# flxrcz/hommx

Measured on AMD Instinct MI355X. Metric: micro-cell solves/sec, higher is better.
Workload: dtype f64

## Files before the change

### hommx_amd/csrc/fused2d.hip

```cpp
#include <hip/hip_runtime.h>
#include <stdint.h>

#include <type_traits>

#include "kernels.h"
#include "sweep_acc.h"

#ifndef HOMMX_FUSED_WAVES_PER_SIMD
#define HOMMX_FUSED_WAVES_PER_SIMD 2
#endif

namespace hommx {

typedef double d4 __attribute__((ext_vector_type(4)));
typedef double d2 __attribute__((ext_vector_type(2)));

__device__ __forceinline__ double uniform_f64(double v) {
  return __hiloint2double(__builtin_amdgcn_readfirstlane(__double2hiint(v)),
                          __builtin_amdgcn_readfirstlane(__double2loint(v)));
}

struct CoefRow {
  double a0, a1;
  double a0m, a1m;
};

constexpr int MATP = 48;

template <int NB>
struct alignas(16) Lds {
  double mat[(NB + 1) * MATP];
  double ubuf[4 * NB];
  double tsc[16 * 17];
  double rrow[2][NB];
  double vrow[2][NB];
  double vnat[2][NB];
  double e0row[NB];
  double e1row[NB];
  double e0nat[NB];
  double e1nat[NB];
  double dgnat[NB];
  double cenat[NB + 2];
};
template <int NB>
struct alignas(16) LdsIso {
  static constexpr int PARK = NB == 32 ? 12 * 64 : 0;
  double ubuf[4 * NB];
  double tsc[16 * 17];
  double rrow[2][NB];
  double vrow[2][NB];
  double vnat[2][NB];
  double e0row[NB];
  double e0nat[NB];
  double dgnat[NB];
  double cenat[NB + 2];
  double park[PARK ? PARK : 1];
};

struct NoFact {};
template <int NB, bool FACT, bool ISO>
__global__ __launch_bounds__(64, (NB == 32 && ISO) ? 3 : HOMMX_FUSED_WAVES_PER_SIMD) void k_poisson2d_fused(
    const double* __restrict__ coef, const double* __restrict__ Mmat, double* __restrict__ out,
    int32_t* __restrict__ info, int n, long long ncells, const CoefSource src, std::conditional_t<FACT, double*, NoFact> fact
#ifdef HOMMX_FUSED_DEBUG
    , double* __restrict__ dbg
#endif
) {
  constexpr int NT = NB / 16, KK = NB / 4, CG = 64 / NB;
  constexpr int P = MATP;
  constexpr bool PARK = ISO && NB == 32;
  static_assert(!(FACT && ISO), "the factor record keeps the general path");
  __shared__ std::conditional_t<ISO, LdsIso<NB>, Lds<NB>> L;

  const long long cell = blockIdx.x;
  if (cell >= ncells) return;
  __builtin_assume(n >= 3);
  __builtin_assume(n <= NB);
  const int l = threadIdx.x;
  const int j = l & 15, k = l >> 4;
  const int c = l % NB, g = l / NB;
  const int lb = l - c;
  const int p0 = NB - n;
  const bool valid = c >= p0;
  const int cn = c - p0;
  const int cm = valid ? (c == p0 ? NB - 1 : c - 1) : c;
  const int cp = valid ? (c == NB - 1 ? p0 : c + 1) : c;
  const int prow = (c & 3) * KK + (c >> 2);

  const int ownB = (k + 1) * P + j;
  [[maybe_unused]] int leftB[NT];
#pragma unroll
  for (int tj = 0; tj < NT; ++tj) {
    const int col = 16 * tj + j;
    leftB[tj] = (k + 1) * P + (col == p0 ? NB - 1 : col - 1);
  }
#define OWN(ti, tj, r) (ownB + (16 * (ti) + 4 * (r)) * P + 16 * (tj))
#define LEFT(ti, tj, r) (leftB[tj] + (16 * (ti) + 4 * (r)) * P)
  [[maybe_unused]] unsigned matOff = 0;
  if constexpr (!ISO) matOff = accl::lds_offset(&L.mat[0]);
  [[maybe_unused]] const unsigned haloA = matOff + 8u * (unsigned)(p0 * P + j);

  const int mode = src.mode;
  const unsigned char* mask = static_cast<const unsigned char*>(src.table);
  const double* table = static_cast<const double*>(src.table);
  const double* cc = mode == COEF_STREAM ? coef + cell * (2ll * n * n) : coef + cell * 2;
  constexpr int NL = NB * NB / 64;
  double2 pv[NL];
  if (mode == COEF_STREAM) {
#pragma unroll
    for (int i = 0; i < NL; ++i) {
      const int el = 2 * l + 128 * i;
      pv[i] = el < 2 * n * n ? *reinterpret_cast<const double2*>(cc + el) : double2{0.0, 0.0};
    }
  }

  if constexpr (!ISO)
    for (int i = l; i < (NB + 1) * P; i += 64) L.mat[i] = 0.0;
  if (l == 0) L.cenat[0] = 0.0;

  double m00 = 1.0, m01 = 0.0, m10 = 0.0, m11 = 1.0;
  if (!ISO && Mmat) {
    const double* mp = Mmat + cell * 4;
    m00 = mp[0]; m01 = mp[1]; m10 = mp[2]; m11 = mp[3];
  }
  const double al = ISO ? 0.5 : uniform_f64(0.5 * (m00 * m00 + m10 * m10));
  const double be = ISO ? 0.5 : uniform_f64(0.5 * (m01 * m01 + m11 * m11));
  const double ga = ISO ? 0.0 : uniform_f64(0.5 * (m00 * m01 + m10 * m11));
  const double ab = ISO ? 1.0 : uniform_f64(al - 2.0 * ga + be);

  double ph0 = 0.0, ph1 = 0.0;
  if (mode != COEF_STREAM) {
    ph0 = cc[0];
    ph1 = cc[1];
  }
  const int nq = src.nq;
  auto sample = [&](long long el) {
    double acc = 0.0;
    for (int q = 0; q < nq; ++q)
      acc = add_rn(acc, mul_rn(src.weights[q], div_rn(1.0, add_rn(ph0, mul_rn(ph1, table[el * nq + q])))));
    return acc;
  };
  auto load_pair = [&](long long el, double& a0, double& a1) {
    if (mode == COEF_TWO_PHASE) {
      const uchar2 mk = *reinterpret_cast<const uchar2*>(mask + el);
      a0 = mk.x ? ph1 : ph0;
      a1 = mk.y ? ph1 : ph0;
    } else if (mode == COEF_AFFINE) {
      const double2 g2 = *reinterpret_cast<const double2*>(table + el);
      a0 = add_rn(ph0, mul_rn(ph1, g2.x));
      a1 = add_rn(ph0, mul_rn(ph1, g2.y));
    } else if (mode == COEF_RECIPROCAL) {
      a0 = sample(el);
      a1 = sample(el + 1);
    } else {
      const double2 v = *reinterpret_cast<const double2*>(cc + el);
      a0 = v.x; a1 = v.y;
    }
  };
  int esh;
  {
    int ef = 0;
    if (mode == COEF_STREAM) {
      int hm = 0;
#pragma unroll
      for (int i = 0; i < NL; ++i) hm = max(hm, max(__double2hiint(pv[i].x) & 0x7fffffff, __double2hiint(pv[i].y) & 0x7fffffff));
      ef = hm >> 20;
    } else {
      for (long long el = 2 * l; el < 2ll * n * n; el += 128) {
        double a0, a1;
        load_pair(el, a0, a1);
        const int f0 = (__double2hiint(a0) >> 20) & 0x7ff, f1 = (__double2hiint(a1) >> 20) & 0x7ff;
        ef = max(ef, max(f0, f1));
      }
    }
#pragma unroll
    for (int off = 32; off >= 1; off >>= 1) ef = max(ef, __shfl_xor(ef, off, 64));
    const int fm = (__double2hiint(6.0 * (al + be)) >> 20) & 0x7ff;
    const int sh = (ef == 0 || ef == 0x7ff ? 0 : ef - 1023) + (fm == 0 || fm == 0x7ff ? 0 : fm - 1023) + 2;
    esh = __builtin_amdgcn_readfirstlane(ef == 0 || ef == 0x7ff ? 0 : sh);
  }
  auto load_row = [&](int jc) {
    CoefRow r;
    r.a0 = 0.0; r.a1 = 0.0;
    if (valid) {
      load_pair(2 * (jc * n + cn), r.a0, r.a1);
      r.a0 = ldexp(r.a0, -esh);
      r.a1 = ldexp(r.a1, -esh);
    }
    r.a0m = __shfl(r.a0, lb + cm, 64);
    r.a1m = __shfl(r.a1, lb + cm, 64);
    return r;
  };
  auto st_diag = [&](const CoefRow& cur, const CoefRow& prev) {
    return valid ? cur.a0 * al + cur.a1 * be + cur.a0m * ab + prev.a0m * be + prev.a1m * al + prev.a1 * ab : 1.0;
  };
  auto st_E = [&](const CoefRow& cur, const CoefRow& prev) { return (cur.a0 + prev.a1) * (ga - al); };
  auto st_N = [&](const CoefRow& cur) { return (cur.a1 + cur.a0m) * (ga - be); };
  auto st_NE = [&](const CoefRow& cur) { return -ga * (cur.a0 + cur.a1); };
  auto st_p0 = [&](const CoefRow& cur, const CoefRow& prev) { return cur.a0 - cur.a0m - prev.a1m + prev.a1; };
  auto st_p1 = [&](const CoefRow& cur, const CoefRow& prev) { return cur.a1 + cur.a0m - prev.a0m - prev.a1; };

  [[maybe_unused]] auto band_write = [&](double dv, double ov, bool sym, bool clear) {
    if constexpr (!ISO) {
      if (g == 0) {
        const double d_ = clear ? 0.0 : dv, o_ = clear ? 0.0 : ov;
        L.mat[(c + 1) * P + c] = d_;
        if (valid) {
          L.mat[(cp + 1) * P + c] = o_;
          if (sym) L.mat[(c + 1) * P + cp] = o_;
        }
      }
    }
  };
  auto sub_band = [&](double (&x)[NT][NT][4], const double (&dgq)[NT], const double (&ceq)[NT], const double (&cemq)[NT]) {
#pragma unroll
    for (int t = 0; t < NT; ++t) {
      using namespace accl;
#define DIAG_LO(r) (OneLane<0, 4 * (r)>::lo | OneLane<1, 4 * (r) + 1>::lo | OneLane<2, 4 * (r) + 2>::lo | OneLane<3, 4 * (r) + 3>::lo)
#define DIAG_HI(r) (OneLane<0, 4 * (r)>::hi | OneLane<1, 4 * (r) + 1>::hi | OneLane<2, 4 * (r) + 2>::hi | OneLane<3, 4 * (r) + 3>::hi)
      masked_sub4<DIAG_LO(0), DIAG_HI(0), DIAG_LO(1), DIAG_HI(1), DIAG_LO(2), DIAG_HI(2), DIAG_LO(3), DIAG_HI(3)>(
          x[t][t][0], x[t][t][1], x[t][t][2], x[t][t][3], dgq[t]);
#define SUB_LO(r) (((r) ? OneLane<0, (4 * (r) - 1) & 15>::lo : 0u) | OneLane<1, 4 * (r)>::lo | OneLane<2, 4 * (r) + 1>::lo | OneLane<3, 4 * (r) + 2>::lo)
#define SUB_HI(r) (((r) ? OneLane<0, (4 * (r) - 1) & 15>::hi : 0u) | OneLane<1, 4 * (r)>::hi | OneLane<2, 4 * (r) + 1>::hi | OneLane<3, 4 * (r) + 2>::hi)
      masked_sub4<SUB_LO(0), SUB_HI(0), SUB_LO(1), SUB_HI(1), SUB_LO(2), SUB_HI(2), SUB_LO(3), SUB_HI(3)>(
          x[t][t][0], x[t][t][1], x[t][t][2], x[t][t][3], ceq[t]);
#define SUP_LO(r) (OneLane<0, 4 * (r) + 1>::lo | OneLane<1, 4 * (r) + 2>::lo | OneLane<2, 4 * (r) + 3>::lo | ((r) < 3 ? OneLane<3, (4 * (r) + 4) & 15>::lo : 0u))
#define SUP_HI(r) (OneLane<0, 4 * (r) + 1>::hi | OneLane<1, 4 * (r) + 2>::hi | OneLane<2, 4 * (r) + 3>::hi | ((r) < 3 ? OneLane<3, (4 * (r) + 4) & 15>::hi : 0u))
      masked_sub4<SUP_LO(0), SUP_HI(0), SUP_LO(1), SUP_HI(1), SUP_LO(2), SUP_HI(2), SUP_LO(3), SUP_HI(3)>(
          x[t][t][0], x[t][t][1], x[t][t][2], x[t][t][3], cemq[t]);
#undef DIAG_LO
#undef DIAG_HI
#undef SUB_LO
#undef SUB_HI
#undef SUP_LO
#undef SUP_HI
    }
    if (NT == 2) {
      using namespace accl;
      masked_sub<OneLane<0, 15>::lo, OneLane<0, 15>::hi>(x[NT - 1][0][0], ceq[0]);
      masked_sub<OneLane<3, 0>::lo, OneLane<3, 0>::hi>(x[0][NT - 1][3], cemq[NT - 1]);
    }
  };
  [[maybe_unused]] auto band_regs = [&](double (&x)[NT][NT][4], double dv, double ov) {
    double dq[NT], oq[NT], omq[NT];
#pragma unroll
    for (int tj = 0; tj < NT; ++tj) {
      const int col = 16 * tj + j;
      dq[tj] = __shfl(dv, col, 64);
      oq[tj] = __shfl(ov, col, 64);
      const double om = __shfl(ov, (col + 63) & 63, 64);
      omq[tj] = col == 0 ? 0.0 : om;
    }
#pragma unroll
    for (int ti = 0; ti < NT; ++ti)
#pragma unroll
      for (int tj = 0; tj < NT; ++tj)
#pragma unroll
        for (int r = 0; r < 4; ++r) x[ti][tj][r] = 0.0;
    sub_band(x, dq, oq, omq);
    const double cw = readlane_f64(ov, NB - 1);
#pragma unroll
    for (int tj = 0; tj < NT; ++tj) x[NT - 1][tj][3] = (k == 3 && 16 * tj + j == p0) ? x[NT - 1][tj][3] - cw : x[NT - 1][tj][3];
#pragma unroll
    for (int ti = 0; ti < NT; ++ti)
#pragma unroll
      for (int r = 0; r < 4; ++r) x[ti][NT - 1][r] = (j == 15 && 16 * ti + 4 * r + k == p0) ? x[ti][NT - 1][r] - cw : x[ti][NT - 1][r];
  };

  [[maybe_unused]] double* rec = nullptr;
  if constexpr (FACT) rec = fact + cell * fused_fact_doubles(n);
  [[maybe_unused]] double* srec = nullptr;
  if constexpr (FACT) srec = rec + fused_fact_header(NB);

  double wf[NT][KK];
  double a[NT][NT][4];
  d4 slr[NT][NT];
  double rr[2];
  double rlm;
  CoefRow cur;
  double asum;
  __syncthreads();
  {
    const CoefRow rowA = load_row(n - 2);
    const CoefRow rowB = load_row(n - 1);
    cur = load_row(0);
    asum = (rowB.a0 + rowB.a1) + (cur.a0 + cur.a1);
    if constexpr (FACT) {
      const double neB = st_NE(rowB);
      const double c1 = __shfl(neB, lb + cm, 64);
      if (g == 0) {
        rec[c] = st_N(rowB);
        rec[NB + c] = c1;
      }
      if (l < 4) rec[4 * NB + l] = l == 0 ? m00 : l == 1 ? m01 : l == 2 ? m10 : m11;
      if (l == 4) rec[4 * NB + 4] = (double)esh;
    }
    if constexpr (ISO) {
      band_regs(a, -st_diag(rowB, rowA), -st_E(rowB, rowA));
#pragma unroll
      for (int ti = 0; ti < NT; ++ti)
#pragma unroll
        for (int tj = 0; tj <= ti; ++tj)
#pragma unroll
          for (int r = 0; r < 4; ++r) slr[ti][tj][r] = a[ti][tj][r];
      if constexpr (PARK) {
#pragma unroll
        for (int ti = 0; ti < NT; ++ti)
#pragma unroll
          for (int tj = 0; tj <= ti; ++tj)
#pragma unroll
            for (int r = 0; r < 4; ++r) L.park[(4 * (ti * (ti + 1) / 2 + tj) + r) * 64 + l] = slr[ti][tj][r];
      }
      band_regs(a, st_diag(cur, rowB), st_E(cur, rowB));
      const double dv = st_N(rowB);
#pragma unroll
      for (int t = 0; t < NT; ++t) {
        using namespace accl;
#pragma unroll
        for (int kk = 0; kk < KK; ++kk) wf[t][kk] = 0.0;
        const double dq = __shfl(dv, 16 * t + j, 64);
        amov<DiagMask<0>::lo, DiagMask<0>::hi>(wf[t][4 * t], dq);
        amov<DiagMask<1>::lo, DiagMask<1>::hi>(wf[t][4 * t + 1], dq);
        amov<DiagMask<2>::lo, DiagMask<2>::hi>(wf[t][4 * t + 2], dq);
        amov<DiagMask<3>::lo, DiagMask<3>::hi>(wf[t][4 * t + 3], dq);
      }
    } else {
    {
      const double dv = st_diag(rowB, rowA), ov = st_E(rowB, rowA);
      band_write(dv, ov, true, false);
      __syncthreads();
#pragma unroll
      for (int ti = 0; ti < NT; ++ti)
#pragma unroll
        for (int tj = 0; tj <= ti; ++tj)
#pragma unroll
          for (int r = 0; r < 4; ++r) slr[ti][tj][r] = L.mat[OWN(ti, tj, r)];
      __syncthreads();
      band_write(dv, ov, true, true);
      __syncthreads();
    }
    {
      const double dv = st_N(rowB), ov = st_NE(rowB);
      band_write(dv, ov, false, false);
      __syncthreads();
#pragma unroll
      for (int t = 0; t < NT; ++t)
#pragma unroll
        for (int kk = 0; kk < KK; ++kk) wf[t][kk] = L.mat[OWN(kk >> 2, t, kk & 3)];
      __syncthreads();
      band_write(dv, ov, false, true);
      __syncthreads();
    }
    {
      const double dv = -st_diag(cur, rowB), ov = -st_E(cur, rowB);
      band_write(dv, ov, true, false);
      __syncthreads();
#pragma unroll
      for (int ti = 0; ti < NT; ++ti)
#pragma unroll
        for (int tj = 0; tj < NT; ++tj)
#pragma unroll
          for (int r = 0; r < 4; ++r) a[ti][tj][r] = L.mat[OWN(ti, tj, r)];
      __syncthreads();
      band_write(dv, ov, true, true);
      __syncthreads();
    }
    }
    rr[0] = st_p0(cur, rowB); rr[1] = st_p1(cur, rowB);
    rlm = (k >> 1) ? st_p1(rowB, rowA) : st_p0(rowB, rowA);
  }
  double ga_ = 0.0, gb_ = 0.0;
  int bad = 0, badstep = 0;
  [[maybe_unused]] double wselR[NT];
#pragma unroll
  for (int tj = 0; tj < NT; ++tj) wselR[tj] = (k == 3 && 16 * tj + j == p0) ? 1.0 : 0.0;
  [[maybe_unused]] const double wselC = (j == 15 && k == (p0 & 3)) ? 1.0 : 0.0;
  [[maybe_unused]] const int laneR = 48 + (p0 & 15), tileR = p0 >> 4, laneC = 16 * (p0 & 3) + 15;
  double indw[KK];
#pragma unroll
  for (int q = 0; q < KK; ++q) indw[q] = uniform_f64((q == (p0 >> 2)) ? 1.0 : 0.0);

  for (int jr = 0; jr <= n - 2; ++jr) {
    const bool lastStep = (jr == n - 2);
    CoefRow nxt = cur;
    if (!lastStep) {
      nxt = load_row(jr + 1);
      asum += nxt.a0 + nxt.a1;
    }
    const double e0c = st_N(cur);
    [[maybe_unused]] double neC = 0.0, e1c = 0.0;
    if constexpr (!ISO) {
      neC = st_NE(cur);
      e1c = __shfl(neC, lb + cm, 64);
    }
    if (lastStep) {
      if constexpr (ISO) {
#pragma unroll
        for (int t = 0; t < NT; ++t) {
          using namespace accl;
          const double me = -__shfl(e0c, 16 * t + j, 64);
          masked_sub4<DiagMask<0>::lo, DiagMask<0>::hi, DiagMask<1>::lo, DiagMask<1>::hi, DiagMask<2>::lo, DiagMask<2>::hi, DiagMask<3>::lo,
                      DiagMask<3>::hi>(wf[t][4 * t], wf[t][4 * t + 1], wf[t][4 * t + 2], wf[t][4 * t + 3], me);
        }
      } else {
        for (int i = l; i < (NB + 1) * P; i += 64) L.mat[i] = 0.0;
        __syncthreads();
        if (g == 0) {
          L.mat[(c + 1) * P + c] = e0c;
          if (valid) L.mat[(c + 1) * P + cp] = neC;
        }
        __syncthreads();
#pragma unroll
        for (int t = 0; t < NT; ++t)
#pragma unroll
          for (int kk = 0; kk < KK; ++kk) wf[t][kk] += L.mat[OWN(kk >> 2, t, kk & 3)];
        __syncthreads();
      }
    }
    [[maybe_unused]] double pn0 = 0.0, pn1 = 0.0;
    if constexpr (ISO) {
      pn0 = st_p0(nxt, cur);
      pn1 = st_p1(nxt, cur);
    }
    const double dgc = st_diag(nxt, cur), cec = st_E(nxt, cur);
    if (g == 0) {
      L.rrow[0][prow] = rr[0];
      L.rrow[1][prow] = rr[1];
      L.e0row[prow] = e0c;
      if constexpr (!ISO) L.e1row[prow] = e1c;
      L.e0nat[c] = e0c;
      if constexpr (!ISO) L.e1nat[c] = e1c;
      L.dgnat[c] = dgc;
      L.cenat[1 + c] = cec;
    }

    {
      int badj = 0;
#ifdef HOMMX_FUSED_SWEEP32
      accl::Sweep<NB>::run(a, L.ubuf, j, k, badj);
#else
      __builtin_amdgcn_s_setprio(1);
      if constexpr (NB == 32) accl::block_inverse32(a, L.ubuf, L.tsc, j, k, badj);
      else accl::Sweep<NB>::run(a, L.ubuf, j, k, badj);
      __builtin_amdgcn_s_setprio(0);
#endif
      if (badj && !bad) { bad = 1; badstep = jr + 1; }
    }
    if constexpr (FACT) {
#pragma unroll
      for (int ti = 0; ti < NT; ++ti)
#pragma unroll
        for (int tj = 0; tj < NT; ++tj)
#pragma unroll
          for (int r = 0; r < 4; ++r) srec[((ti * NT + tj) * 4 + r) * 64 + l] = a[ti][tj][r];
      if (g == 0) {
        srec[NB * NB + 2 * NB + c] = e0c;
        srec[NB * NB + 3 * NB + c] = e1c;
      }
    }
#ifdef HOMMX_FUSED_DEBUG
    if (dbg && cell == 0) {
      double* q = dbg + (size_t)jr * 4 * NB * NB;
#pragma unroll
      for (int ti = 0; ti < NT; ++ti)
#pragma unroll
        for (int tj = 0; tj < NT; ++tj)
#pragma unroll
          for (int r = 0; r < 4; ++r) q[(16 * ti + 4 * r + k) * NB + 16 * tj + j] = a[ti][tj][r];
#pragma unroll
      for (int t = 0; t < NT; ++t)
#pragma unroll
        for (int kk = 0; kk < KK; ++kk) q[NB * NB + (16 * t + j) * NB + 4 * kk + k] = wf[t][kk];
    }
#endif

    if constexpr (!ISO) if (!lastStep) {
#pragma unroll
      for (int ti = 0; ti < NT; ++ti)
#pragma unroll
        for (int tj = 0; tj < NT; ++tj)
#pragma unroll
          for (int r = 0; r < 4; ++r) L.mat[OWN(ti, tj, r)] = a[ti][tj][r];
#pragma unroll
      for (int tj = 0; tj < NT; ++tj)
        accl::masked_lds_store<accl::RowMask<3>::lo, accl::RowMask<3>::hi>(haloA + 128u * tj, a[NT - 1][tj][3]);
    }

    d4 vt[NT][NT];
#pragma unroll
    for (int x = 0; x < NT; ++x)
#pragma unroll
      for (int y = 0; y < NT; ++y) vt[x][y] = d4{0.0, 0.0, 0.0, 0.0};
#pragma unroll
    for (int kk = 0; kk < KK; ++kk)
#pragma unroll
      for (int x = 0; x < NT; ++x)
#pragma unroll
        for (int y = 0; y < NT; ++y)
          vt[x][y] = __builtin_amdgcn_mfma_f64_16x16x4f64(a[kk >> 2][x][kk & 3], wf[y][kk], vt[x][y], 0, 0, 0);

    if constexpr (PARK) {
#pragma unroll
      for (int x = 0; x < NT; ++x)
#pragma unroll
        for (int y = 0; y <= x; ++y) {
          double* pk = &L.park[4 * (x * (x + 1) / 2 + y) * 64 + l];
          d4 s;
#pragma unroll
          for (int r = 0; r < 4; ++r) s[r] = pk[64 * r];
#pragma unroll
          for (int kk = 0; kk < KK; ++kk) s = __builtin_amdgcn_mfma_f64_16x16x4f64(vt[kk >> 2][x][kk & 3], wf[y][kk], s, 0, 0, 0);
#pragma unroll
          for (int r = 0; r < 4; ++r) pk[64 * r] = s[r];
        }
    } else {
#pragma unroll
    for (int kk = 0; kk < KK; ++kk)
#pragma unroll
      for (int x = 0; x < NT; ++x)
#pragma unroll
        for (int y = 0; y <= x; ++y)
          slr[x][y] = __builtin_amdgcn_mfma_f64_16x16x4f64(vt[kk >> 2][x][kk & 3], wf[y][kk], slr[x][y], 0, 0, 0);
    }

    double z;
    {
      double part[2][NT];
#pragma unroll
      for (int m = 0; m < 2; ++m)
#pragma unroll
        for (int tj = 0; tj < NT; ++tj) part[m][tj] = 0.0;
#pragma unroll
      for (int m = 0; m < 2; ++m)
#pragma unroll
        for (int ti = 0; ti < NT; ++ti) {
          const d4 q = *reinterpret_cast<const d4*>(&L.rrow[m][k * KK + 4 * ti]);
#pragma unroll
          for (int r = 0; r < 4; ++r)
#pragma unroll
            for (int tj = 0; tj < NT; ++tj) part[m][tj] = fma(q[r], a[ti][tj][r], part[m][tj]);
        }
      if (NT == 2) {
        double s_[2];
#pragma unroll
        for (int m = 0; m < 2; ++m) {
          double x = part[m][0], y = part[m][NT - 1];
          swap16(x, y);
          s_[m] = x + y;
        }
        swap32(s_[0], s_[1]);
        z = s_[0] + s_[1];
      } else {
        double x = part[0][0], y = part[1][0];
        swap32(x, y);
        z = add_xor16(x + y);
      }
    }
    if constexpr (ISO) {
      ga_ = fma(z, L.rrow[0][prow], ga_);
      gb_ = fma(z, L.rrow[1][prow], gb_);
    } else {
      ga_ = fma(z, rr[0], ga_);
      gb_ = fma(z, rr[1], gb_);
    }
    L.vnat[k >> 1][c] = z;
    L.vrow[k >> 1][prow] = z;
    if constexpr (FACT) {
      if (NB == 32 || !(k & 1)) srec[NB * NB + (k >> 1) * NB + c] = z;
      srec += fused_fact_step(NB);
    }

    {
      double part[2][NT];
#pragma unroll
      for (int m = 0; m < 2; ++m) {
        double v[KK];
#pragma unroll
        for (int q4 = 0; q4 < KK; q4 += 4) {
          const d4 q = *reinterpret_cast<const d4*>(&L.vrow[m][k * KK + q4]);
          v[q4] = q[0]; v[q4 + 1] = q[1]; v[q4 + 2] = q[2]; v[q4 + 3] = q[3];
        }
#pragma unroll
        for (int t = 0; t < NT; ++t) {
          double acc = 0.0;
#pragma unroll
          for (int kk = 0; kk < KK; ++kk) acc = fma(v[kk], wf[t][kk], acc);
          part[m][t] = acc;
        }
      }
      double z6;
      if (NT == 2) {
        double s_[2];
#pragma unroll
        for (int m = 0; m < 2; ++m) {
          double x = part[m][0], y = part[m][NT - 1];
          swap16(x, y);
          s_[m] = x + y;
        }
        swap32(s_[0], s_[1]);
        z6 = s_[0] + s_[1];
      } else {
        double x = part[0][0], y = part[1][0];
        swap32(x, y);
        z6 = add_xor16(x + y);
      }
      rlm += z6;
    }

    if (!lastStep) {
      [[maybe_unused]] double e0r[KK];
      [[maybe_unused]] double e1r[KK];
#pragma unroll
      for (int q4 = 0; q4 < KK; q4 += 4) {
        if constexpr (!ISO) {
          const d4 x = *reinterpret_cast<const d4*>(&L.e0row[k * KK + q4]);
          const d4 y = *reinterpret_cast<const d4*>(&L.e1row[k * KK + q4]);
          e0r[q4] = x[0]; e0r[q4 + 1] = x[1]; e0r[q4 + 2] = x[2]; e0r[q4 + 3] = x[3];
          e1r[q4] = y[0]; e1r[q4 + 1] = y[1]; e1r[q4 + 2] = y[2]; e1r[q4 + 3] = y[3];
        }
      }
      {
        double e0q[NT], dgq[NT], ceq[NT], cemq[NT];
        [[maybe_unused]] double e1q[NT];
#pragma unroll
        for (int tj = 0; tj < NT; ++tj) {
          e0q[tj] = L.e0nat[16 * tj + j];
          if constexpr (!ISO) e1q[tj] = L.e1nat[16 * tj + j];
          dgq[tj] = L.dgnat[16 * tj + j];
          ceq[tj] = L.cenat[1 + 16 * tj + j];
          cemq[tj] = L.cenat[16 * tj + j];
        }
#pragma unroll
        for (int ti = 0; ti < NT; ++ti)
#pragma unroll
          for (int r = 0; r < 4; ++r)
#pragma unroll
            for (int tj = 0; tj < NT; ++tj) {
              if constexpr (ISO) {
                a[ti][tj][r] = -(L.e0row[k * KK + 4 * ti + r] * (e0q[tj] * a[ti][tj][r]));
              } else {
                const double nl = L.mat[LEFT(ti, tj, r)];
                const double nu = L.mat[OWN(ti, tj, r) - P];
                const double nul = L.mat[LEFT(ti, tj, r) - P];
                const double x = fma(e1q[tj], nl, e0q[tj] * a[ti][tj][r]);
                const double xu = fma(e1q[tj], nul, e0q[tj] * nu);
                a[ti][tj][r] = -fma(e0r[4 * ti + r], x, e1r[4 * ti + r] * xu);
              }
            }
        sub_band(a, dgq, ceq, cemq);
        {
          const double cw = readlane_f64(cec, NB - 1);
#pragma unroll
          for (int tj = 0; tj < NT; ++tj) {
            if constexpr (ISO) a[NT - 1][tj][3] = (l == laneR && tj == tileR) ? fma(-cw, 1.0, a[NT - 1][tj][3]) : fma(-cw, 0.0, a[NT - 1][tj][3]);
            else a[NT - 1][tj][3] = fma(-cw, wselR[tj], a[NT - 1][tj][3]);
          }
          double vcol;
          if constexpr (ISO) vcol = l == laneC ? -cw : -cw * 0.0;
          else vcol = -cw * wselC;
#pragma unroll
          for (int ti = 0; ti < NT; ++ti)
#pragma unroll
            for (int r = 0; r < 4; ++r) a[ti][NT - 1][r] = fma(vcol, indw[4 * ti + r], a[ti][NT - 1][r]);
        }
      }

      if constexpr (ISO) {
#pragma unroll
        for (int kk = 0; kk < KK; ++kk)
#pragma unroll
          for (int t = 0; t < NT; ++t) wf[t][kk] = L.e0row[k * KK + kk] * vt[kk >> 2][t][kk & 3];
      } else {
#pragma unroll
        for (int x = 0; x < NT; ++x)
#pragma unroll
          for (int y = 0; y < NT; ++y)
#pragma unroll
            for (int r = 0; r < 4; ++r) L.mat[OWN(x, y, r)] = vt[x][y][r];
#pragma unroll
        for (int y = 0; y < NT; ++y)
          accl::masked_lds_store<accl::RowMask<3>::lo, accl::RowMask<3>::hi>(haloA + 128u * y, vt[NT - 1][y][3]);
#pragma unroll
        for (int t = 0; t < NT; ++t)
#pragma unroll
          for (int kk = 0; kk < KK; ++kk) {
            const double up = L.mat[OWN(kk >> 2, t, kk & 3) - P];
            wf[t][kk] = fma(e1r[kk], up, e0r[kk] * vt[kk >> 2][t][kk & 3]);
          }
      }

      {
        const double v0 = L.vnat[0][c], v1 = L.vnat[1][c];
        if constexpr (ISO) {
          const double e0 = L.e0nat[c];
          rr[0] = fma(v0, e0, pn0);
          rr[1] = fma(v1, e0, pn1);
        } else {
          const double vm0 = L.vnat[0][cm], vm1 = L.vnat[1][cm];
          rr[0] = fma(vm0, e1c, fma(v0, e0c, st_p0(nxt, cur)));
          rr[1] = fma(vm1, e1c, fma(v1, e0c, st_p1(nxt, cur)));
        }
      }
      cur = nxt;
      __syncthreads();
    }
  }

  int lt = l, jt = j, kt = k, ct = c, prowt = prow;
  if constexpr (ISO) {
    lt = (int)__lane_id();
    asm volatile("" : "+v"(lt));
    jt = lt & 15;
    kt = lt >> 4;
    ct = lt % NB;
    prowt = (ct & 3) * KK + (ct >> 2);
  }
  {
  const int l = lt, j = jt, k = kt, c = ct, prow = prowt;
  [[maybe_unused]] auto bfly = [&](double v, int off) {
    const int ad = (l ^ off) << 2;
    return __hiloint2double(__builtin_amdgcn_ds_bpermute(ad, __double2hiint(v)), __builtin_amdgcn_ds_bpermute(ad, __double2loint(v)));
  };
  {
    if constexpr (PARK) {
#pragma unroll
      for (int ti = 0; ti < NT; ++ti)
#pragma unroll
        for (int tj = 0; tj <= ti; ++tj)
#pragma unroll
          for (int r = 0; r < 4; ++r) slr[ti][tj][r] = L.park[(4 * (ti * (ti + 1) / 2 + tj) + r) * 64 + l];
    }
    [[maybe_unused]] d4 sup = d4{0.0, 0.0, 0.0, 0.0};
    if (NT == 2) {
      if constexpr (ISO) {
        sup = accl::transpose_tile(slr[NT - 1][0], L.tsc, j, k);
      } else {
#pragma unroll
        for (int r = 0; r < 4; ++r) L.mat[OWN(1, 0, r)] = slr[NT - 1][0][r];
        __syncthreads();
      }
    }
#pragma unroll
    for (int ti = 0; ti < NT; ++ti)
#pragma unroll
      for (int tj = 0; tj < NT; ++tj)
#pragma unroll
        for (int r = 0; r < 4; ++r) {
          if (tj <= ti) a[ti][tj][r] = -slr[ti][tj][r];
          else if constexpr (ISO) a[ti][tj][r] = -sup[r];
          else a[ti][tj][r] = -L.mat[(16 + j + 1) * P + 4 * r + k];
        }
    {
      using namespace accl;
#pragma unroll
      for (int tj = 0; tj < NT; ++tj) amov<RowMask<3>::lo, RowMask<3>::hi>(a[NT - 1][tj][3], 0.0);
#pragma unroll
      for (int ti = 0; ti < NT; ++ti)
#pragma unroll
        for (int r = 0; r < 4; ++r) amov<ColMask<15>::lo, ColMask<15>::hi>(a[ti][NT - 1][r], 0.0);
      amov<OneLane<3, 15>::lo, OneLane<3, 15>::hi>(a[NT - 1][NT - 1][3], -1.0);
    }
    if (c == NB - 1) rlm = 0.0;
    __syncthreads();
    L.rrow[k >> 1][prow] = rlm;
    L.vnat[k >> 1][c] = rlm;
    __syncthreads();
    int badj = 0;
    accl::Sweep<NB>::run(a, L.ubuf, j, k, badj);
    if (badj && !bad) { bad = 1; badstep = n; }
    if constexpr (FACT) {
#pragma unroll
      for (int ti = 0; ti < NT; ++ti)
#pragma unroll
        for (int tj = 0; tj < NT; ++tj)
#pragma unroll
          for (int r = 0; r < 4; ++r) srec[((ti * NT + tj) * 4 + r) * 64 + l] = a[ti][tj][r];
    }
    double part[2][NT];
#pragma unroll
    for (int m = 0; m < 2; ++m)
#pragma unroll
      for (int tj = 0; tj < NT; ++tj) part[m][tj] = 0.0;
#pragma unroll
    for (int m = 0; m < 2; ++m)
#pragma unroll
      for (int ti = 0; ti < NT; ++ti) {
        const d4 q = *reinterpret_cast<const d4*>(&L.rrow[m][k * KK + 4 * ti]);
#pragma unroll
        for (int r = 0; r < 4; ++r)
#pragma unroll
          for (int tj = 0; tj < NT; ++tj) part[m][tj] = fma(q[r], a[ti][tj][r], part[m][tj]);
      }
    double z;
    if (NT == 2) {
      double s_[2];
#pragma unroll
      for (int m = 0; m < 2; ++m) {
        double x = part[m][0], y = part[m][NT - 1];
        swap16(x, y);
        s_[m] = x + y;
      }
      swap32(s_[0], s_[1]);
      z = s_[0] + s_[1];
    } else {
      double x = part[0][0], y = part[1][0];
      swap32(x, y);
      z = add_xor16(x + y);
    }
    ga_ = fma(z, L.vnat[0][c], ga_);
    gb_ = fma(z, L.vnat[1][c], gb_);
    if constexpr (FACT) {
      if (NB == 32 || !(k & 1)) rec[2 * NB + (k >> 1) * NB + c] = z;
    }
  }

  double g00 = (k < 2) ? ga_ : 0.0, g01 = (k < 2) ? gb_ : 0.0, g11 = (k < 2) ? 0.0 : gb_;
#pragma unroll
  for (int off = 32; off >= 1; off >>= 1) {
    if constexpr (ISO) {
      g00 += bfly(g00, off);
      g01 += bfly(g01, off);
      g11 += bfly(g11, off);
      asum += bfly(asum, off);
    } else {
      g00 += __shfl_xor(g00, off, 64);
      g01 += __shfl_xor(g01, off, 64);
      g11 += __shfl_xor(g11, off, 64);
      asum += __shfl_xor(asum, off, 64);
    }
  }
  if (l == 0) {
    const double h = 1.0 / n;
    constexpr int DUP = 32 / NB;
    const double sc = 0.25 * h * h / DUP;
    const double c0 = 0.5 * h * h * asum / CG;
    const double t00 = m00 * g00 + m01 * g01, t01 = m00 * g01 + m01 * g11;
    const double t10 = m10 * g00 + m11 * g01, t11 = m10 * g01 + m11 * g11;
    double* o = out + cell * 4;
    o[0] = ldexp(c0 + sc * (t00 * m00 + t01 * m01), esh);
    o[1] = ldexp(sc * (t00 * m10 + t01 * m11), esh);
    o[2] = ldexp(sc * (t10 * m00 + t11 * m01), esh);
    o[3] = ldexp(c0 + sc * (t10 * m10 + t11 * m11), esh);
    if (info) info[cell] = bad ? badstep : 0;
  }
  }
#undef OWN
#undef LEFT
}

#ifndef HOMMX_DEV_LDS_PAD
#define HOMMX_DEV_LDS_PAD 0
#endif
#ifdef HOMMX_FUSED_DEBUG
extern double* g_fused_dbg;
#define HOMMX_FUSED_LDS 0
#define HOMMX_FUSED_DBG_ARG , g_fused_dbg
#else
#define HOMMX_FUSED_LDS HOMMX_DEV_LDS_PAD
#define HOMMX_FUSED_DBG_ARG
#endif

#if defined(HOMMX_FUSED_ISO_TU)
hipError_t launch_poisson2d_fused_iso(const double* d_coef, double* d_out, int32_t* d_info, int n, long long ncells, hipStream_t stream,
                                      CoefSource src) {
  if (ncells <= 0) return hipSuccess;
  dim3 grid((unsigned)ncells), block(64);
  const double* d_M = nullptr;
  if (n <= 16)
    hipLaunchKernelGGL((k_poisson2d_fused<16, false, true>), grid, block, HOMMX_FUSED_LDS, stream, d_coef, d_M, d_out, d_info, n, ncells, src,
                       NoFact{} HOMMX_FUSED_DBG_ARG);
  else
    hipLaunchKernelGGL((k_poisson2d_fused<32, false, true>), grid, block, HOMMX_FUSED_LDS, stream, d_coef, d_M, d_out, d_info, n, ncells, src,
                       NoFact{} HOMMX_FUSED_DBG_ARG);
  return hipGetLastError();
}

#elif !defined(HOMMX_FUSED_FACT_TU)
hipError_t launch_poisson2d_fused(const double* d_coef, const double* d_M, double* d_out, int32_t* d_info,
                                  int n, long long ncells, hipStream_t stream, CoefSource src) {
  if (ncells <= 0) return hipSuccess;
  if (!d_M) return launch_poisson2d_fused_iso(d_coef, d_out, d_info, n, ncells, stream, src);
  dim3 grid((unsigned)ncells), block(64);
  if (n <= 16)
    hipLaunchKernelGGL((k_poisson2d_fused<16, false, false>), grid, block, HOMMX_FUSED_LDS, stream, d_coef, d_M, d_out, d_info, n, ncells, src,
                       NoFact{} HOMMX_FUSED_DBG_ARG);
  else
    hipLaunchKernelGGL((k_poisson2d_fused<32, false, false>), grid, block, HOMMX_FUSED_LDS, stream, d_coef, d_M, d_out, d_info, n, ncells, src,
                       NoFact{} HOMMX_FUSED_DBG_ARG);
  return hipGetLastError();
}

#else
hipError_t launch_poisson2d_fused_fact(const double* d_coef, const double* d_M, double* d_out, int32_t* d_info, int n, long long ncells,
                                       hipStream_t stream, double* d_fact) {
  if (ncells <= 0) return hipSuccess;
  dim3 grid((unsigned)ncells), block(64);
  const CoefSource src;
  if (n <= 16)
    hipLaunchKernelGGL((k_poisson2d_fused<16, true, false>), grid, block, 0, stream, d_coef, d_M, d_out, d_info, n, ncells, src,
                       d_fact HOMMX_FUSED_DBG_ARG);
  else
    hipLaunchKernelGGL((k_poisson2d_fused<32, true, false>), grid, block, 0, stream, d_coef, d_M, d_out, d_info, n, ncells, src,
                       d_fact HOMMX_FUSED_DBG_ARG);
  return hipGetLastError();
}
#endif

}
```

Measured before the change: 8.402 million.

## Close first iso step analytically, special-case unpadded wrap, park asum in LDS

For the isotropic path, the first elimination step's W is diagonal. The Schur update is therefore computed as a direct elementwise scaling instead of MFMA products. When the cell is unpadded (p0==0), the periodic-wrap correction becomes two single-lane masked subtracts instead of loops over tiles. In the NB=32 parked variant, the running coefficient sum moves to LDS to free a register. This adds branches and extra LDS traffic in exchange for fewer MFMA and FMA operations and lower register pressure.

After: 8.488 million, median of 6. 1.0% higher.

```diff
diff --git a/hommx_amd/csrc/fused2d.hip b/hommx_amd/csrc/fused2d.hip
--- a/hommx_amd/csrc/fused2d.hip
+++ b/hommx_amd/csrc/fused2d.hip
@@ -8,6 +8,12 @@
 
 #ifndef HOMMX_FUSED_WAVES_PER_SIMD
 #define HOMMX_FUSED_WAVES_PER_SIMD 2
+#endif
+#ifndef HOMMX_ISO_STEP0_CLOSED
+#define HOMMX_ISO_STEP0_CLOSED 1
+#endif
+#ifndef HOMMX_ISO_WRAP_UNPADDED
+#define HOMMX_ISO_WRAP_UNPADDED 1
 #endif
 
 namespace hommx {
@@ -55,6 +61,7 @@
   double dgnat[NB];
   double cenat[NB + 2];
   double park[PARK ? PARK : 1];
+  double asum[PARK ? 64 : 1];
 };
 
 struct NoFact {};
@@ -69,6 +76,8 @@
   constexpr int NT = NB / 16, KK = NB / 4, CG = 64 / NB;
   constexpr int P = MATP;
   constexpr bool PARK = ISO && NB == 32;
+  constexpr bool STEP0 = ISO && HOMMX_ISO_STEP0_CLOSED;
+  constexpr bool WRAPU = ISO && HOMMX_ISO_WRAP_UNPADDED;
   static_assert(!(FACT && ISO), "the factor record keeps the general path");
   __shared__ std::conditional_t<ISO, LdsIso<NB>, Lds<NB>> L;
 
@@ -279,6 +288,7 @@
   double rlm;
   CoefRow cur;
   double asum;
+  [[maybe_unused]] double w0 = 0.0;
   __syncthreads();
   {
     const CoefRow rowA = load_row(n - 2);
@@ -324,6 +334,7 @@
         amov<DiagMask<2>::lo, DiagMask<2>::hi>(wf[t][4 * t + 2], dq);
         amov<DiagMask<3>::lo, DiagMask<3>::hi>(wf[t][4 * t + 3], dq);
       }
+      w0 = dv;
     } else {
     {
       const double dv = st_diag(rowB, rowA), ov = st_E(rowB, rowA);
@@ -380,12 +391,20 @@
 #pragma unroll
   for (int q = 0; q < KK; ++q) indw[q] = uniform_f64((q == (p0 >> 2)) ? 1.0 : 0.0);
 
+  if constexpr (PARK) L.asum[l] = asum;
+  if constexpr (STEP0) {
+    if (g == 0) {
+      L.vnat[0][c] = w0;
+      L.vrow[0][prow] = w0;
+    }
+  }
   for (int jr = 0; jr <= n - 2; ++jr) {
     const bool lastStep = (jr == n - 2);
     CoefRow nxt = cur;
     if (!lastStep) {
       nxt = load_row(jr + 1);
-      asum += nxt.a0 + nxt.a1;
+      if constexpr (PARK) L.asum[l] += nxt.a0 + nxt.a1;
+      else asum += nxt.a0 + nxt.a1;
     }
     const double e0c = st_N(cur);
     [[maybe_unused]] double neC = 0.0, e1c = 0.0;
@@ -487,6 +506,34 @@
     }
 
     d4 vt[NT][NT];
+    bool first = false;
+    if constexpr (STEP0) first = jr == 0;
+    if (first) {
+      if constexpr (STEP0) {
+#pragma unroll
+        for (int y = 0; y < NT; ++y) {
+          const double wq = L.vnat[0][16 * y + j];
+#pragma unroll
+          for (int x = y; x < NT; ++x) {
+            [[maybe_unused]] double* pk = nullptr;
+            if constexpr (PARK) pk = &L.park[4 * (x * (x + 1) / 2 + y) * 64 + l];
+#pragma unroll
+            for (int r = 0; r < 4; ++r) {
+              const double vw = a[x][y][r] * L.vrow[0][k * KK + 4 * x + r];
+              if constexpr (PARK) pk[64 * r] = fma(vw, wq, pk[64 * r]);
+              else slr[x][y][r] = fma(vw, wq, slr[x][y][r]);
+            }
+          }
+#pragma unroll
+          for (int x = 0; x < NT; ++x) {
+            d4 nt = d4{a[x][y][0], a[x][y][1], a[x][y][2], a[x][y][3]};
+            if (x == y) nt = accl::transpose_tile(nt, L.tsc, j, k);
+#pragma unroll
+            for (int r = 0; r < 4; ++r) vt[x][y][r] = nt[r] * wq;
+          }
+        }
+      }
+    } else {
 #pragma unroll
     for (int x = 0; x < NT; ++x)
 #pragma unroll
@@ -521,6 +568,7 @@
 #pragma unroll
         for (int y = 0; y <= x; ++y)
           slr[x][y] = __builtin_amdgcn_mfma_f64_16x16x4f64(vt[kk >> 2][x][kk & 3], wf[y][kk], slr[x][y], 0, 0, 0);
+    }
     }
 
     double z;
@@ -648,7 +696,14 @@
               }
             }
         sub_band(a, dgq, ceq, cemq);
-        {
+        bool unpadded = false;
+        if constexpr (WRAPU) unpadded = p0 == 0;
+        if (unpadded) {
+          using namespace accl;
+          const double cw = readlane_f64(cec, NB - 1);
+          masked_sub<OneLane<3, 0>::lo, OneLane<3, 0>::hi>(a[NT - 1][0][3], cw);
+          masked_sub<OneLane<0, 15>::lo, OneLane<0, 15>::hi>(a[0][NT - 1][0], cw);
+        } else {
           const double cw = readlane_f64(cec, NB - 1);
 #pragma unroll
           for (int tj = 0; tj < NT; ++tj) {
@@ -717,6 +772,7 @@
   }
   {
   const int l = lt, j = jt, k = kt, c = ct, prow = prowt;
+  if constexpr (PARK) asum = L.asum[l];
   [[maybe_unused]] auto bfly = [&](double v, int off) {
     const int ad = (l ^ off) << 2;
     return __hiloint2double(__builtin_amdgcn_ds_bpermute(ad, __double2hiint(v)), __builtin_amdgcn_ds_bpermute(ad, __double2loint(v)));
```
